# wuxiaolang/Cube_SLAM_wu

Measured on AMD Instinct MI355X. Metric: frames/sec detect_cuboid, higher is better.
Workload: dtype f64

## Files before the change

### cube_slam_wu_amd/csrc/detect_kernels.hip

```cpp
#include <hip/hip_runtime.h>
#include "cs_hip_util.h"

#include <cstdio>
#include <cstdlib>
#include <cstring>

#include "../../include/cubeslam_hip.h"
#include "detect_types.h"
#include "cs_atan2_lean.h"

namespace cs {

__device__ __forceinline__ int wave_uniform_i32(int x) { return __builtin_amdgcn_readfirstlane(x); }
__device__ __forceinline__ long long wave_uniform_i64(long long x) {
  const unsigned lo = (unsigned)__builtin_amdgcn_readfirstlane((int)(unsigned)(x & 0xffffffffll)), hi = (unsigned)__builtin_amdgcn_readfirstlane((int)(x >> 32));
  return (long long)(((unsigned long long)hi << 32) | lo);
}
__device__ __forceinline__ double wave_uniform_f64(double x) {
  int lo, hi;
  asm("v_readfirstlane_b32 %0, %1" : "=s"(lo) : "v"(__double2loint(x)));
  asm("v_readfirstlane_b32 %0, %1" : "=s"(hi) : "v"(__double2hiint(x)));
  return __hiloint2double(hi, lo);
}
template <typename T>
__device__ __forceinline__ int find_job_wave(const T* __restrict__ prefix, int n, T elem) {
  const T first = sizeof(T) == 8 ? (T)wave_uniform_i64((long long)elem) : (T)wave_uniform_i32((int)elem);
  int lo = 0, hi = n;
  while (hi - lo > 1) {
    const int mid = (lo + hi) >> 1;
    if (prefix[mid] <= first) lo = mid; else hi = mid;
  }
  while (lo + 1 < n && prefix[lo + 1] <= elem) lo++;
  return lo;
}

__device__ __forceinline__ long long xcd_virtual_block() {
  long long nb = gridDim.x, b = blockIdx.x;
  return (b & 7) * (nb >> 3) + (b >> 3);
}

__device__ __attribute__((noinline)) double vp_exact_raw(double dy, double dx) { return cs_atan2(dy, dx); }

__device__ __forceinline__ double vp_exact_unwrapped(const double* __restrict__ mx, const double* __restrict__ my, int i, int ib, double vpxk, double vpyk) {
  const double raw = vp_exact_raw(my[i] - vpyk, mx[i] - vpxk);
  if (i == ib) return raw;
  const double base = vp_exact_raw(my[ib] - vpyk, mx[ib] - vpxk);
  if ((raw - base) < -CS_PI) return raw + 2 * CS_PI;
  if ((raw - base) > CS_PI) return raw - 2 * CS_PI;
  return raw;
}
__device__ __attribute__((noinline)) float vp_rare_unwrapped_f(const double* mx, const double* my, int i, int ib, double vpxk, double vpyk) {
  return (float)vp_exact_unwrapped(mx, my, i, ib, vpxk, vpyk);
}
__device__ __attribute__((noinline)) bool vp_rare_greater(const double* mx, const double* my, int i, int i_ref, int ib, double vpxk, double vpyk) {
  return vp_exact_unwrapped(mx, my, i, ib, vpxk, vpyk) > vp_exact_unwrapped(mx, my, i_ref, ib, vpxk, vpyk);
}
__device__ __attribute__((noinline)) bool vp_rare_less(const double* mx, const double* my, int i, int i_ref, int ib, double vpxk, double vpyk) {
  return vp_exact_unwrapped(mx, my, i, ib, vpxk, vpyk) < vp_exact_unwrapped(mx, my, i_ref, ib, vpxk, vpyk);
}
struct VpExactInlier { float at; int inl; };
__device__ __attribute__((noinline)) VpExactInlier vp_rare_inlier(double dyd, double dxd, double lai, double thre) {
  const double raw = cs_atan2(dyd, dxd);
  const double nrm = normalize_to_pi(raw);
  double d = dabs(lai - nrm);
  d = dmin(d, CS_PI - d);
  return VpExactInlier{(float)raw, d < thre ? 1 : 0};
}

struct VpRun {
  bool have;
  int ib, i_hi, i_lo;
  float base_f, hi_f, lo_f;
  double hx, hy, lx, ly;
};

__device__ __forceinline__ float atan2_float(float fy, float fx, bool* usable) {
  const float PI_F = 3.14159274f, HPI_F = 1.57079637f;
  const float ay = fabsf(fy), ax = fabsf(fx);
  const float hi = fmaxf(ax, ay), lo = fminf(ax, ay);
  const float q = lo * __builtin_amdgcn_rcpf(hi), q2 = q * q;
  float at = -0.01172120f;
  at = __builtin_fmaf(at, q2, 0.05265332f);
  at = __builtin_fmaf(at, q2, -0.11643287f);
  at = __builtin_fmaf(at, q2, 0.19354346f);
  at = __builtin_fmaf(at, q2, -0.33262347f);
  at = __builtin_fmaf(at, q2, 0.99997726f);
  at = at * q;
  if (ay > ax) at = HPI_F - at;
  if (fx < 0.0f) at = PI_F - at;
  if (fy < 0.0f) at = -at;
  *usable = hi > 0.0f && hi < 3.0e38f;
  return at;
}

__device__ __forceinline__ void vp_step(const double* __restrict__ mx, const double* __restrict__ my, int i, double mxi, double myi, double lai,
                                        double vpxk, double vpyk, double thre, float thre_f, VpRun& R) {
  const float PI_F = 3.14159274f, HPI_F = 1.57079637f, M_IN = 1.0e-5f, M_ORD = 2.0e-5f;
  const double dyd = myi - vpyk, dxd = mxi - vpxk;
  bool usable;
  float at = atan2_float((float)dyd, (float)dxd, &usable);
  float nr = at;
  if (at > HPI_F) nr = at - PI_F; else if (at < -HPI_F) nr = at + PI_F;
  float df = fabsf((float)lai - nr);
  df = fminf(df, PI_F - df);
  bool inl = usable && df < thre_f - M_IN;
  if (!(inl || (usable && df > thre_f + M_IN))) { const VpExactInlier x = vp_rare_inlier(dyd, dxd, lai, thre); inl = x.inl != 0; at = x.at; }
  if (inl) {
    if (!R.have) {
      R.have = true; R.ib = i; R.i_hi = i; R.i_lo = i; R.base_f = at; R.hi_f = at; R.lo_f = at; R.hx = dxd; R.hy = dyd; R.lx = dxd; R.ly = dyd;
    } else {
      const float d = at - R.base_f;
      float sh = d < -PI_F ? at + 2.0f * PI_F : d > PI_F ? at - 2.0f * PI_F : at;
      if (fabsf(fabsf(d) - PI_F) < M_ORD) sh = vp_rare_unwrapped_f(mx, my, i, R.ib, vpxk, vpyk);
      if (sh > R.hi_f + M_ORD) { R.hi_f = sh; R.i_hi = i; R.hx = dxd; R.hy = dyd; }
      else if (sh > R.hi_f - M_ORD) {
        const double c = R.hx * dyd - R.hy * dxd, lim = 1.0e-12 * ((dabs(dxd) + dabs(dyd)) * (dabs(R.hx) + dabs(R.hy)));
        const bool greater = c > lim ? true : c < -lim ? false : vp_rare_greater(mx, my, i, R.i_hi, R.ib, vpxk, vpyk);
        if (greater) { R.hi_f = sh; R.i_hi = i; R.hx = dxd; R.hy = dyd; }
      }
      if (sh < R.lo_f - M_ORD) { R.lo_f = sh; R.i_lo = i; R.lx = dxd; R.ly = dyd; }
      else if (sh < R.lo_f + M_ORD) {
        const double c = R.lx * dyd - R.ly * dxd, lim = 1.0e-12 * ((dabs(dxd) + dabs(dyd)) * (dabs(R.lx) + dabs(R.ly)));
        const bool less = c < -lim ? true : c > lim ? false : vp_rare_less(mx, my, i, R.i_lo, R.ib, vpxk, vpyk);
        if (less) { R.lo_f = sh; R.i_lo = i; R.lx = dxd; R.ly = dyd; }
      }
    }
  }
}

struct VpChunk {
  double2 xy[64];
  double ang[64];
  float2 dir[64];
};

template <int K, bool UNIFORM>
__device__ __forceinline__ void vp_support_multi(const double* __restrict__ mx, const double* __restrict__ my, const double* __restrict__ la, int m, VpChunk* ch,
                                                 const double* vpx, const double* vpy, const double* thre, const bool* swapped, bool lane_on, double* out) {
  VpRun R[K];
  float thre_f[K], tan_f[K];
#pragma unroll
  for (int k = 0; k < K; k++) {
    R[k] = VpRun{false, 0, 0, 0, 0.f, 0.f, 0.f, 0., 0., 0., 0.}; thre_f[k] = (float)thre[k];
    tan_f[k] = thre_f[k] < 1.5f ? tanf(thre_f[k] + 1.0e-4f) : __builtin_huge_valf();
  }
  if (UNIFORM) {
    const int lane = threadIdx.x & 63;
    for (int c0 = 0; c0 < m; c0 += 64) {
      const int n = min(64, m - c0);
      __builtin_amdgcn_fence(__ATOMIC_ACQ_REL, "wavefront");
      if (lane < n) {
        const double a = la[c0 + lane];
        ch->xy[lane] = make_double2(mx[c0 + lane], my[c0 + lane]);
        ch->ang[lane] = a;
        ch->dir[lane] = make_float2(cosf((float)a), sinf((float)a));
      }
      __builtin_amdgcn_fence(__ATOMIC_ACQ_REL, "wavefront");
      __builtin_amdgcn_wave_barrier();
// ... 165 lines not shown
  int flag = 0;
  int j = find_job_wave<long long>(v.slot_prefix, v.n_jobs, active ? tid : slot_total - 1);
  const int ju = wave_uniform_i32(j);
  if (__all(j == ju)) {
    if (active) flag = candidate_one(v, sp, v.jobs[ju], tid);
  } else {
    if (active) flag = candidate_one(v, sp, v.jobs[j], tid);
  }
  unsigned long long valid = __ballot(flag != 0);
  if (valid) {
    int lane = threadIdx.x & 63;
    int j0 = __shfl(j, __ffsll((long long)valid) - 1);
    unsigned long long same = __ballot(flag != 0 && j == j0);
    if (same == valid) {
      if (lane == __ffsll((long long)valid) - 1) atomicAdd(&v.job_valid[j0], __popcll(valid));
    } else if (flag != 0) {
      atomicAdd(&v.job_valid[j], 1);
    }
  }
}

enum { COMPACT_PER = 16 };
enum { CC_TRIP = 4096 };
__global__ __launch_bounds__(256) void candidate_compact_kernel(DetectDeviceView v, SweepParams sp) {
  const int j = blockIdx.x;
  if (j >= v.n_jobs) return;
  __shared__ unsigned char s_flag[CC_TRIP];
  __shared__ int wsum[4];
  const int tid = threadIdx.x, lane = tid & 63, wid = tid >> 6;
  int jd_Y, jd_T, jd_rp_off, jd_yaw_off, jd_vp_off, jd_top_off, n_vp;
  BoxGeomD gd;
  {
    const JobDesc& jd = v.jobs[j];
    jd_Y = jd.Y; jd_T = jd.T; jd_rp_off = jd.rp_off; jd_yaw_off = jd.yaw_off; jd_vp_off = jd.vp_off; jd_top_off = jd.top_off;
    n_vp = jd.RP * jd.Y;
    const BoxGeomD g = box_geom_d(jd.g);
    gd = BoxGeomD{g.left, wave_uniform_f64(g.top), g.right, wave_uniform_f64(g.down),
                  wave_uniform_f64(g.el), wave_uniform_f64(g.et), wave_uniform_f64(g.er), wave_uniform_f64(g.eb)};
  }
  int* out_valid = v.job_valid + j;
  long long* out_cbase = v.job_cbase + j;
  asm volatile("" : "+v"(out_valid), "+v"(out_cbase));
  for (int e = tid; e < n_vp; e += 256) {
    const int rp = e / jd_Y, y = e - rp * jd_Y;
    const RpPose* pose = v.rp + jd_rp_off + rp;
    const double cy = v.yaw_cos[jd_yaw_off + y], sy = v.yaw_sin[jd_yaw_off + y];
    const double* A = pose->KinvR;
    const double d[3][3] = {{cy, sy, 0.0}, {-sy, cy, 0.0}, {0.0, 0.0, 1.0}};
    double* vout = v.vp + 6 * (long long)(jd_vp_off + e);
#pragma unroll
    for (int k = 0; k < 3; k++) {
      const double h0 = (A[0] * d[k][0] + A[1] * d[k][1]) + A[2] * d[k][2];
      const double h1 = (A[3] * d[k][0] + A[4] * d[k][1]) + A[5] * d[k][2];
      const double h2 = (A[6] * d[k][0] + A[7] * d[k][1]) + A[8] * d[k][2];
      vout[2 * k] = h0 / h2;
      vout[2 * k + 1] = h1 / h2;
    }
  }
  __syncthreads();
  const unsigned half = (unsigned)n_vp * (unsigned)jd_T;
  const unsigned Tu = (unsigned)jd_T;
  const bool fast_div = Tu > 1 && (unsigned long long)half * Tu < (1ull << 32);
  const unsigned inv_T = fast_div ? 0xffffffffu / Tu + 1u : 0u;
  const long long base = v.slot_prefix[j];
  long long run = base;
  const unsigned long long below = (1ull << lane) - 1ull;
  const bool en1 = sp.consider_config_1 != 0, en2 = sp.consider_config_2 != 0;
  const double* job_vp = v.vp + 6 * (long long)jd_vp_off;
  const int* job_top_x = v.top_x + jd_top_off;
  for (unsigned r0 = 0; r0 < half; r0 += CC_TRIP / 2) {
#pragma unroll 1
    for (int q = 0; q < 16; q++) {
      const int cfg = 1 + (q >> 3);
      const unsigned rl = (unsigned)(q & 7) * 256u + (unsigned)tid, rest = r0 + rl;
      int flag = 0;
      if (rest < half && (cfg == 1 ? en1 : en2)) {
        const unsigned ryu = fast_div ? __umulhi(rest, inv_T) : rest / Tu;
        const int t = (int)(rest - ryu * Tu);
        const double* vp = job_vp + 6 * (long long)(int)ryu;
        V2 c[8];
        flag = build_corners(gd, v2(vp[0], vp[1]), v2(vp[2], vp[3]), v2(vp[4], vp[5]), (double)job_top_x[t], cfg, sp.short_sq_bound, c);
      }
      s_flag[2 * rl + (unsigned)(cfg - 1)] = (unsigned char)flag;
    }
    __syncthreads();
    int f[COMPACT_PER];
    int wcount = 0;
#pragma unroll
    for (int q = 0; q < COMPACT_PER; q++) {
      f[q] = s_flag[wid * (64 * COMPACT_PER) + q * 64 + lane];
      wcount += __popcll(__ballot(f[q] != 0));
    }
    if (lane == 0) wsum[wid] = wcount;
    __syncthreads();
    int woff = 0, total = 0;
#pragma unroll
    for (int w = 0; w < 4; w++) { const int x = wsum[w]; if (w < wid) woff += x; total += x; }
    long long pos0 = run + woff;
    const long long sl0 = base + 2ll * r0 + wid * (64 * COMPACT_PER) + lane;
#pragma unroll
    for (int q = 0; q < COMPACT_PER; q++) {
      const unsigned long long bal = __ballot(f[q] != 0);
      if (f[q] != 0) {
        const long long pos = pos0 + __popcll(bal & below);
        v.c_slot[pos] = sl0 + q * 64;
        v.c_flag[pos] = f[q] | (j << CAND_JOB_SHIFT);
      }
      pos0 += __popcll(bal);
    }
    run += total;
    __syncthreads();
  }
  const int n_valid = (int)(run - base);
  if (tid == 0) { *out_valid = n_valid; *out_cbase = base; }
  const int nblk = (n_valid + 255) >> 8;
  if (nblk > 0) {
    __shared__ int s_at;
    if (tid == 0) s_at = atomicAdd(&v.blk_info[0], nblk);
    __syncthreads();
    const int at = s_at, b0 = (int)(base >> 8);
    for (int k = tid; k < nblk; k += 256) {
      const int left = n_valid - 256 * k;
      v.blk_info[2 + 2 * (long long)(at + k)] = b0 + k;
      v.blk_info[3 + 2 * (long long)(at + k)] = left > 256 ? 256 : left;
    }
  }
}

__device__ __forceinline__ int slot_corners(const DetectDeviceView& v, const JobDesc& jd, long long slot, double short_sq_bound, V2 c[8]) {
  const unsigned local = (unsigned)(slot - jd.slot_off);
  const unsigned rest = local >> 1, ryu = rest / (unsigned)jd.T;
  const int t = (int)(rest - ryu * (unsigned)jd.T);
  const double* vp = v.vp + 6 * (long long)(jd.vp_off + (int)ryu);
  return build_corners(jd.g, v2(vp[0], vp[1]), v2(vp[2], vp[3]), v2(vp[4], vp[5]), (double)v.top_x[jd.top_off + t], (int)(local & 1) + 1, short_sq_bound, c);
}
__device__ __forceinline__ void slot_corners16(const DetectDeviceView& v, long long slot, double short_sq_bound, double out16[16]) {
  int lo = 0, hi = v.n_jobs;
  while (hi - lo > 1) { const int mid = (lo + hi) >> 1; if (v.slot_prefix[mid] <= slot) lo = mid; else hi = mid; }
  V2 c[8];
#pragma unroll
  for (int q = 0; q < 8; q++) c[q] = v2(0.0, 0.0);
  slot_corners(v, v.jobs[lo], slot, short_sq_bound, c);
#pragma unroll
  for (int q = 0; q < 8; q++) { out16[q] = c[q].x; out16[8 + q] = c[q].y; }
}

__device__ __forceinline__ int sel(int cfg, int a, int b) { return cfg ? b : a; }

enum { SCORE_JOBS = 4, SCORE_SUB = 128, SCORE_BINS = SCORE_JOBS * SCORE_SUB };
__device__ __forceinline__ unsigned score_udiv(unsigned n, unsigned d, unsigned inv) { return inv ? __umulhi(n, inv) : n / d; }

enum { SCORE_WAVE_MIXED = 0, SCORE_WAVE_CFG1 = 1, SCORE_WAVE_CFG2 = 2 };
__device__ __forceinline__ unsigned score_sample_index(double sy, double sx, int map_w) { return (unsigned)(__mul24((int)sy, map_w) + (int)sx); }
template <int MODE>
__device__ __forceinline__ void score_edge_trip(int e0, int cfg, const double (*CXt)[260], const double (*CYt)[260], int tx, double ox, double oy,
                                                const float* __restrict__ map, int map_w, float& sum_dist) {
  const bool c2 = MODE == SCORE_WAVE_MIXED ? cfg != 0 : MODE == SCORE_WAVE_CFG2;
  const unsigned long long EA = c2 ? 0x004213210ull : 0x443213210ull, EB = c2 ? 0x005450321ull : 0x577450321ull;
  const unsigned long long EW = c2 ? 0x004332222ull : 0x222222222ull;
  const int n_edges = c2 ? 7 : 9;
  constexpr int EU = 3;
  float dv[EU][11];
#pragma unroll
  for (int u = 0; u < EU; u++) {
    const int e = e0 + u;
    if (MODE != SCORE_WAVE_MIXED && e >= n_edges) continue;
    const int a = (int)((EA >> (4 * e)) & 7), b = (int)((EB >> (4 * e)) & 7);
    const double x1 = CXt[a][tx] - ox, y1 = CYt[a][tx] - oy, x2 = CXt[b][tx] - ox, y2 = CYt[b][tx] - oy;
#pragma unroll
    for (int s = 0; s < 11; s++) {
      double sx, sy;
      if (s == 0) { sx = x2; sy = y2; }
      else if (s == 10) { sx = x1; sy = y1; }
      else if (s == 5) { sx = (x1 + x2) * 0.5; sy = (y1 + y2) * 0.5; }
      else { const double w = (double)s / 10.0; sx = w * x1 + (1 - w) * x2; sy = w * y1 + (1 - w) * y2; }
      dv[u][s] = map[score_sample_index(sy, sx, map_w)];
    }
  }
#pragma unroll
  for (int u = 0; u < EU; u++) {
    const int e = e0 + u;
    const float wt = MODE == SCORE_WAVE_CFG1 ? 1.0f : 0.5f * (float)(int)((EW >> (4 * e)) & 7);
    const bool on = e < n_edges;
    if (MODE == SCORE_WAVE_MIXED) {
#pragma unroll
      for (int s = 0; s < 11; s++) { const float nx = sum_dist + dv[u][s] * wt; sum_dist = on ? nx : sum_dist; }
    } else if (!on) {
    } else if (wt == 1.0f) {
#pragma unroll
      for (int s = 0; s < 11; s++) sum_dist += dv[u][s];
    } else {
#pragma unroll
      for (int s = 0; s < 11; s++) sum_dist += dv[u][s] * wt;
    }
  }
}
template <int MODE>
__device__ __forceinline__ float score_edge_sum(int cfg, const double (*CXt)[260], const double (*CYt)[260], int tx, double ox, double oy,
                                                const float* __restrict__ map, int map_w) {
  float sum_dist = 0;
  const int n_edges = MODE == SCORE_WAVE_MIXED ? (cfg ? 7 : 9) : MODE == SCORE_WAVE_CFG2 ? 7 : 9;
#pragma unroll 1
  for (int e0 = 0; e0 < n_edges; e0 += 3) score_edge_trip<MODE>(e0, cfg, CXt, CYt, tx, ox, oy, map, map_w, sum_dist);
  return sum_dist;
}

__device__ __forceinline__ double score_atan2(double dy, double dx, bool* accepted = nullptr) {
  double a;
  const bool ok = cs_atan2_lean(dy, dx, &a);
  if (__builtin_amdgcn_ballot_w64(!ok) != 0) {
    if (!ok) a = cs_atan2(dy, dx);
  }
  if (accepted) *accepted = ok;
  return a;
}

__global__ __launch_bounds__(256) void score_atan2_check_kernel(const double* __restrict__ y, const double* __restrict__ x, int n, double* __restrict__ out, int* __restrict__ accepted) {
  const int i = blockIdx.x * 256 + threadIdx.x;
  if (i >= n) return;
  bool ok;
  out[i] = score_atan2(y[i], x[i], &ok);
  accepted[i] = ok ? 1 : 0;
}
void launch_score_atan2_check(const double* y, const double* x, int n, double* out, int* accepted, hipStream_t st) {
  if (n <= 0) return;
  hipLaunchKernelGGL(score_atan2_check_kernel, dim3((n + 255) / 256), dim3(256), 0, st, y, x, n, out, accepted);
}

__global__ __launch_bounds__(256) void score_sample_index_check_kernel(const double* __restrict__ sy, const double* __restrict__ sx, const int* __restrict__ map_w,
                                                                       const double* __restrict__ a, const double* __restrict__ b, int n, int* __restrict__ index, double* __restrict__ probe) {
  const int i = blockIdx.x * 256 + threadIdx.x;
  if (i >= n) return;
  double pa = a[i];
  const double pb = b[i];
  const unsigned k = score_sample_index(sy[i], sx[i], map_w[i]);
  asm volatile("" : "+v"(pa) : "v"(k));
  index[i] = (int)k;
  probe[i] = pa + pb;
}
void launch_score_sample_index_check(const double* sy, const double* sx, const int* map_w, const double* a, const double* b, int n, int* index, double* probe, hipStream_t st) {
  if (n <= 0) return;
  hipLaunchKernelGGL(score_sample_index_check_kernel, dim3((n + 255) / 256), dim3(256), 0, st, sy, sx, map_w, a, b, n, index, probe);
}

template <bool CAP>
__global__ __launch_bounds__(256) void score_kernel(DetectDeviceView v, long long slot_total, double short_sq_bound) {
  __shared__ double C16[16][260];
  double (*CXt)[260] = C16, (*CYt)[260] = C16 + 8;
  const bool cap = CAP;
  long long n_valid = cap ? 256ll * v.blk_info[0] : v.job_cbase[v.n_jobs];
  const long long per_xcd = ((n_valid + 255) / 256 + 7) / 8;
  const long long kx = blockIdx.x >> 3;
  if (kx >= per_xcd) return;
  long long base = ((long long)(blockIdx.x & 7) * per_xcd + kx) * blockDim.x;
  if (base >= n_valid) return;
  if (cap) {
    const int* entry = v.blk_info + 2 + 2 * (base >> 8);
    base = 256ll * entry[0];
    n_valid = base + entry[1];
  }
  __shared__ int hist[SCORE_BINS + 1];
  __shared__ int s_src[256], s_job[256], s_flag[256];
  __shared__ long long s_slot[256];
  {
    const int t0 = threadIdx.x;
    for (int b = t0; b <= SCORE_BINS; b += 256) hist[b] = 0;
    __syncthreads();
    const long long i0 = base + t0;
    long long slot0 = 0;
    int j0 = 0;
    int flag0 = 0;
    if (i0 < n_valid) { slot0 = v.c_slot[i0]; flag0 = v.c_flag[i0]; j0 = flag0 >> CAND_JOB_SHIFT; }
    s_slot[t0] = slot0; s_job[t0] = j0; s_flag[t0] = flag0 & CAND_VP_MASK;
    __syncthreads();
    int key = SCORE_BINS;
    if (i0 < n_valid) {
      const int jq = CAP ? __builtin_amdgcn_readfirstlane(s_job[0]) : j0;
      const int T0 = v.jobs[jq].T;
      const unsigned loc = (unsigned)(slot0 - v.jobs[jq].slot_off);
      const int jrel = j0 - s_job[0];
      const unsigned hq = loc >> 1;
      const unsigned qT = CAP ? score_udiv(hq, (unsigned)T0, ((unsigned long long)v.jobs[jq].RP * v.jobs[jq].Y * T0 * T0 < (1ull << 32) && T0 > 1) ? 0xffffffffu / (unsigned)T0 + 1u : 0u) : hq / (unsigned)T0;
      const int sub = (int)(loc & 1) * T0 + (int)(hq - qT * (unsigned)T0);
      key = (jrel < SCORE_JOBS && sub < SCORE_SUB) ? jrel * SCORE_SUB + sub : SCORE_BINS - 1;
    }
    const int rank = atomicAdd(&hist[key], 1);
    __syncthreads();
    if (t0 < 64) {
      constexpr int PER = (SCORE_BINS + 1 + 63) / 64;
      int loc_sum = 0, vals[PER];
#pragma unroll
      for (int q = 0; q < PER; q++) { const int b = t0 * PER + q; vals[q] = b <= SCORE_BINS ? hist[b] : 0; loc_sum += vals[q]; }
      int incl = loc_sum;
#pragma unroll
      for (int o = 1; o < 64; o <<= 1) { const int y = __shfl_up(incl, o); if (t0 >= o) incl += y; }
      int run = incl - loc_sum;
#pragma unroll
      for (int q = 0; q < PER; q++) { const int b = t0 * PER + q; if (b <= SCORE_BINS) hist[b] = run; run += vals[q]; }
    }
    __syncthreads();
    s_src[hist[key] + rank] = t0;
    __syncthreads();
  }
  const int mine = s_src[threadIdx.x];
  const JobDesc& jd = v.jobs[CAP ? __builtin_amdgcn_readfirstlane(s_job[0]) : s_job[mine]];
  const long long i = base + mine;
  if (i >= n_valid) return;
  const long long slot = s_slot[mine];
  const unsigned local = (unsigned)(slot - jd.slot_off);
  const int cfg = (int)(local & 1);
  const unsigned inv_T = (CAP && jd.T > 1 && (unsigned long long)jd.RP * jd.Y * jd.T * jd.T < (1ull << 32)) ? 0xffffffffu / (unsigned)jd.T + 1u : 0u;
  const unsigned inv_Y = (CAP && jd.Y > 1 && (unsigned long long)jd.RP * jd.Y * jd.Y < (1ull << 32)) ? 0xffffffffu / (unsigned)jd.Y + 1u : 0u;
  const int ry = (int)score_udiv(local >> 1, (unsigned)jd.T, inv_T);
  const int rp = (int)score_udiv((unsigned)ry, (unsigned)jd.Y, inv_Y);
  const int tx = threadIdx.x;
  const double ox = (double)jd.g.el, oy = (double)jd.g.et;
  const float* __restrict__ map = v.maps + jd.map_off;
  {
    V2 cb[8];
    const unsigned rest = local >> 1;
    const double* vp = v.vp + 6 * (long long)(jd.vp_off + ry);
    rebuild_accepted_corners(jd.g, v2(vp[0], vp[1]), v2(vp[2], vp[3]), v2(vp[4], vp[5]), (double)v.top_x[jd.top_off + (int)(rest - (unsigned)ry * (unsigned)jd.T)], cfg + 1,
                             s_flag[mine], cb);
#pragma unroll
    for (int q = 0; q < 8; q++) { CXt[q][tx] = cb[q].x; CYt[q][tx] = cb[q].y; }
  }
  double bnd[6];
  {
    const double* bound = v.bound + 6 * (long long)(jd.vp_off + ry);
#pragma unroll
    for (int q = 0; q < 6; q++) bnd[q] = bound[q];
  }
  const int map_w = jd.map_w;
  const bool u1 = __all(cfg == 0), u2 = __all(cfg == 1);
  float sum_dist;
  if (u1) sum_dist = score_edge_sum<SCORE_WAVE_CFG1>(cfg, CXt, CYt, tx, ox, oy, map, map_w);
  else if (u2) sum_dist = score_edge_sum<SCORE_WAVE_CFG2>(cfg, CXt, CYt, tx, ox, oy, map, map_w);
  else sum_dist = score_edge_sum<SCORE_WAVE_MIXED>(cfg, CXt, CYt, tx, ox, oy, map, map_w);
  double total = 0;
  const double not_found_penalty = 30.0 / 180.0 * CS_PI * 2;
  const int ID1[3][4] = {{0, 1, 7, 4}, {3, 0, 4, 5}, {3, 7, 1, 5}}, ID2[3][4] = {{0, 1, 2, 3}, {3, 0, 4, 5}, {2, 4, 1, 5}};
#pragma unroll
  for (int k = 0; k < 3; k++) {
    double b0 = bnd[2 * k], b1 = bnd[2 * k + 1];
    bool v0 = !(b0 != b0), v1 = !(b1 != b1);
    if (v0 || v1) {
#pragma unroll
      for (int ee = 0; ee < 2; ee++) {
        int pa = sel(cfg, ID1[k][2 * ee], ID2[k][2 * ee]), pb = sel(cfg, ID1[k][2 * ee + 1], ID2[k][2 * ee + 1]);
        double ang = normalize_to_pi(score_atan2(CYt[pb][tx] - CYt[pa][tx], CXt[pb][tx] - CXt[pa][tx]));
        double best = 100;
        if (v0) { double t = dabs(ang - b0); t = dmin(t, CS_PI - t); if (t < best) best = t; }
        if (v1) { double t = dabs(ang - b1); t = dmin(t, CS_PI - t); if (t < best) best = t; }
        total = total + best;
      }
    } else {
      total = total + not_found_penalty;
    }
  }
  V2 c[8];
#pragma unroll
  for (int q = 0; q < 8; q++) c[q] = v2(CXt[q][tx], CYt[q][tx]);
  const RpPose* pose = v.rp + jd.rp_off + rp;
  double p3[3], s3[3];
  lift_to_3d(c, pose->R, pose->t, v.invK + 9 * jd.frame, pose->plane, p3, s3);
  int flag = s_flag[mine];
  if (s3[0] < 0 || s3[1] < 0 || s3[2] < 0) flag |= CAND_NEG_SCALE;
  v.c_flag[i] = flag;
  v.c_dist[i] = (double)sum_dist / jd.diag;
  v.c_angle[i] = total;
  v.c_skew[i] = dmax(s3[0], s3[1]) / dmin(s3[0], s3[1]);
}

__global__ __launch_bounds__(1024) void scan_jobs_kernel(const int* job_valid, long long* job_cbase, int n_jobs) {
  __shared__ long long wsum[16];
  __shared__ long long carry_s;
  if (threadIdx.x == 0) carry_s = 0;
  __syncthreads();
  int lane = threadIdx.x & 63, wid = threadIdx.x >> 6;
  for (int base = 0; base < n_jobs; base += 1024) {
    int i = base + threadIdx.x;
    long long x = (i < n_jobs) ? job_valid[i] : 0;
    long long incl = x;
#pragma unroll
    for (int o = 1; o < 64; o <<= 1) {
      long long y = __shfl_up(incl, o);
      if (lane >= o) incl += y;
    }
    if (lane == 63) wsum[wid] = incl;
    __syncthreads();
    long long woff = 0;
    for (int w = 0; w < wid; w++) woff += wsum[w];
    long long carry = carry_s;
    if (i < n_jobs) job_cbase[i] = carry + woff + incl - x;
    __syncthreads();
    if (threadIdx.x == 1023) carry_s = carry + woff + incl;
    __syncthreads();
  }
  if (threadIdx.x == 0) job_cbase[n_jobs] = carry_s;
}

__global__ __launch_bounds__(256) void compact_kernel(DetectDeviceView v) {
  int j = blockIdx.x;
  if (j >= v.n_jobs) return;
  __shared__ int wsum[4];
  const long long s0 = v.slot_prefix[j], s1 = v.slot_prefix[j + 1];
  long long run = v.job_cbase[j];
  const int lane = threadIdx.x & 63, wid = threadIdx.x >> 6;
  const unsigned long long below = (1ull << lane) - 1ull;
  for (long long base = s0; base < s1; base += 256 * COMPACT_PER) {
    const long long w0 = base + (long long)wid * (64 * COMPACT_PER) + lane;
    int f[COMPACT_PER];
    int wcount = 0;
#pragma unroll
    for (int q = 0; q < COMPACT_PER; q++) {
      const long long sl = w0 + q * 64;
      f[q] = (sl < s1) ? v.flag[sl] : 0;
      wcount += __popcll(__ballot(f[q] != 0));
    }
    if (lane == 0) wsum[wid] = wcount;
    __syncthreads();
    int woff = 0, total = 0;
#pragma unroll
    for (int w = 0; w < 4; w++) { const int x = wsum[w]; if (w < wid) woff += x; total += x; }
    long long pos0 = run + woff;
#pragma unroll
    for (int q = 0; q < COMPACT_PER; q++) {
      const unsigned long long bal = __ballot(f[q] != 0);
      if (f[q] != 0) {
        const long long pos = pos0 + __popcll(bal & below);
        v.c_slot[pos] = w0 + q * 64;
        v.c_flag[pos] = f[q] | (j << CAND_JOB_SHIFT);
      }
      pos0 += __popcll(bal);
    }
    run += total;
    __syncthreads();
  }
}

__global__ __launch_bounds__(256) void compact_count_kernel(DetectDeviceView v, int* __restrict__ cnt, int maxc) {
  const int j = blockIdx.x, c = blockIdx.y;
  __shared__ int wsum[4];
  const long long end = v.slot_prefix[j + 1], s0 = v.slot_prefix[j] + (long long)c * (256 * COMPACT_PER), s1 = (s0 + 256 * COMPACT_PER < end) ? s0 + 256 * COMPACT_PER : end;
  int n = 0;
  for (long long sl = s0 + threadIdx.x; sl < s1; sl += 256) n += v.flag[sl] != 0;
#pragma unroll
  for (int o = 32; o > 0; o >>= 1) n += __shfl_down(n, o);
  if ((threadIdx.x & 63) == 0) wsum[threadIdx.x >> 6] = n;
  __syncthreads();
  if (threadIdx.x == 0) cnt[(size_t)j * maxc + c] = wsum[0] + wsum[1] + wsum[2] + wsum[3];
}
__global__ __launch_bounds__(256) void compact_chunk_kernel(DetectDeviceView v, const int* __restrict__ cnt, int maxc) {
  const int j = blockIdx.x, c = blockIdx.y;
  __shared__ int wsum[4];
  const long long s1 = v.slot_prefix[j + 1], base = v.slot_prefix[j] + (long long)c * (256 * COMPACT_PER);
  if (base >= s1) return;
  long long run = v.job_cbase[j];
  for (int q = 0; q < c; q++) run += cnt[(size_t)j * maxc + q];
  const int lane = threadIdx.x & 63, wid = threadIdx.x >> 6;
  const unsigned long long below = (1ull << lane) - 1ull;
  const long long w0 = base + (long long)wid * (64 * COMPACT_PER) + lane;
  int f[COMPACT_PER];
  int wcount = 0;
#pragma unroll
  for (int q = 0; q < COMPACT_PER; q++) {
    const long long sl = w0 + q * 64;
    f[q] = (sl < s1) ? v.flag[sl] : 0;
    wcount += __popcll(__ballot(f[q] != 0));
  }
  if (lane == 0) wsum[wid] = wcount;
  __syncthreads();
  int woff = 0;
#pragma unroll
  for (int w = 0; w < 4; w++) if (w < wid) woff += wsum[w];
  long long pos0 = run + woff;
#pragma unroll
  for (int q = 0; q < COMPACT_PER; q++) {
    const unsigned long long bal = __ballot(f[q] != 0);
    if (f[q] != 0) {
      const long long pos = pos0 + __popcll(bal & below);
      v.c_slot[pos] = w0 + q * 64;
      v.c_flag[pos] = f[q] | (j << CAND_JOB_SHIFT);
    }
    pos0 += __popcll(bal);
  }
}

__global__ __launch_bounds__(64) void gather_corners_kernel(DetectDeviceView v, double short_sq_bound, const long long* slots, int n, double* out) {
  int w = blockIdx.x * blockDim.x + threadIdx.x;
  if (w >= n) return;
  long long s = slots[w];
  double c16[16];
#pragma unroll
  for (int q = 0; q < 16; q++) c16[q] = 0.0;
  if (s >= 0) slot_corners16(v, s, short_sq_bound, c16);
#pragma unroll
  for (int q = 0; q < 16; q++) out[16 * (size_t)w + q] = c16[q];
}


__device__ __forceinline__ unsigned long long order_key(double x) {
  unsigned long long b = (unsigned long long)__double_as_longlong(x);
  return (b >> 63) ? ~b : (b | 0x8000000000000000ull);
}

template <int NT>
__device__ void block_radix_select2(const double* __restrict__ a, const double* __restrict__ b, int n, int r, unsigned* hist , unsigned long long* bcast ,
                                    unsigned long long* key_a, unsigned long long* key_b) {
  unsigned long long prefix[2] = {0, 0}, mask = 0;
  int rr2[2] = {r, r};
  for (int pass = 0; pass < 8; pass++) {
    const int shift = 56 - 8 * pass;
    for (int q = threadIdx.x; q < 512; q += NT) hist[q] = 0;
    __syncthreads();
    for (int i = threadIdx.x; i < n; i += NT) {
      const unsigned long long ka = order_key(a[i]), kb = order_key(b[i]);
      if ((ka & mask) == prefix[0]) atomicAdd(&hist[(unsigned)(ka >> shift) & 255u], 1u);
      if ((kb & mask) == prefix[1]) atomicAdd(&hist[256 + ((unsigned)(kb >> shift) & 255u)], 1u);
// ... 1228 lines not shown
```

Before: 575,600.

## Shrink score kernel LDS footprint and dedupe corner map samples for higher occupancy

Stores corner y-values for corners 0 and 4 as wave-uniform scalars (top/down) rather than in shared memory, cutting corner rows from 16 to 14. In CAP mode it also shrinks the histogram, slot, job and flag arrays. Uniform-config paths are fully unrolled per edge group, with each corner's map sample loaded once and reused as the shared edge endpoint. Launch bounds request five waves in CAP mode, and the bound loads move after the edge sum. The changes rely on the geometric invariant that those corners share top/down y, and add register pressure and complexity.

```diff
diff --git a/cube_slam_wu_amd/csrc/detect_kernels.hip b/cube_slam_wu_amd/csrc/detect_kernels.hip
--- a/cube_slam_wu_amd/csrc/detect_kernels.hip
+++ b/cube_slam_wu_amd/csrc/detect_kernels.hip
@@ -4,6 +4,7 @@
 #include <cstdio>
 #include <cstdlib>
 #include <cstring>
+#include <type_traits>
 
 #include "../../include/cubeslam_hip.h"
 #include "detect_types.h"
@@ -475,41 +476,106 @@
 
 enum { SCORE_WAVE_MIXED = 0, SCORE_WAVE_CFG1 = 1, SCORE_WAVE_CFG2 = 2 };
 __device__ __forceinline__ unsigned score_sample_index(double sy, double sx, int map_w) { return (unsigned)(__mul24((int)sy, map_w) + (int)sx); }
-template <int MODE>
-__device__ __forceinline__ void score_edge_trip(int e0, int cfg, const double (*CXt)[260], const double (*CYt)[260], int tx, double ox, double oy,
-                                                const float* __restrict__ map, int map_w, float& sum_dist) {
-  const bool c2 = MODE == SCORE_WAVE_MIXED ? cfg != 0 : MODE == SCORE_WAVE_CFG2;
-  const unsigned long long EA = c2 ? 0x004213210ull : 0x443213210ull, EB = c2 ? 0x005450321ull : 0x577450321ull;
-  const unsigned long long EW = c2 ? 0x004332222ull : 0x222222222ull;
+
+enum { SCORE_LD = 260, SCORE_XROWS = 8, SCORE_YROWS = 6, SCORE_ROWS = SCORE_XROWS + SCORE_YROWS };
+enum { SCORE_WAVES = 5 };
+enum { SCORE_TOP = -1, SCORE_DOWN = -2 };
+__host__ __device__ constexpr int score_xrow(int c) { return c; }
+__host__ __device__ constexpr int score_yrow(int c) { return c == 0 ? (int)SCORE_TOP : c == 4 ? (int)SCORE_DOWN : SCORE_XROWS + c - 1 - (c > 4 ? 1 : 0); }
+__device__ __forceinline__ double score_uniform_f64(double x) {
+  int lo, hi;
+  asm("s_nop 0\n\tv_readfirstlane_b32 %0, %2\n\tv_readfirstlane_b32 %1, %3\n\ts_nop 1" : "=s"(lo), "=s"(hi) : "v"(__double2loint(x)), "v"(__double2hiint(x)));
+  return __hiloint2double(hi, lo);
+}
+struct ScoreCorners {
+  double (*R)[SCORE_LD];
+  int tx;
+  double top, down;
+  __device__ __forceinline__ double row(int r) const { return r == SCORE_TOP ? +top : r == SCORE_DOWN ? +down : +R[r][tx]; }
+  __device__ __forceinline__ double x(int c) const { return row(score_xrow(c)); }
+  __device__ __forceinline__ double y(int c) const { return row(score_yrow(c)); }
+  __device__ __forceinline__ double pick(int r1, int r2, int cfg) const { return r1 == r2 ? row(r1) : (r1 >= 0 && r2 >= 0) ? +R[cfg ? r2 : r1][tx] : cfg ? row(r2) : row(r1); }
+  __device__ __forceinline__ double x_of(int c1, int c2, int cfg) const { return pick(score_xrow(c1), score_xrow(c2), cfg); }
+  __device__ __forceinline__ double y_of(int c1, int c2, int cfg) const { return pick(score_yrow(c1), score_yrow(c2), cfg); }
+  __device__ __forceinline__ double x_dyn(int c) const { return R[c][tx]; }
+  __device__ __forceinline__ double y_dyn(int c) const {
+    const double s = R[SCORE_XROWS + (c == 0 || c == 4 ? 0 : c - 1 - (c > 4 ? 1 : 0))][tx], t = top, d = down;
+    return c == 0 ? +t : c == 4 ? +d : +s;
+  }
+  template <int Q>
+  __device__ __forceinline__ void store_corner(const V2& p) {
+    if (score_yrow(Q) >= 0) R[score_yrow(Q)][tx] = p.y;
+    R[score_xrow(Q)][tx] = p.x;
+  }
+  __device__ __forceinline__ void store(const V2 (&cb)[8]) {
+    store_corner<0>(cb[0]); store_corner<1>(cb[1]); store_corner<2>(cb[2]); store_corner<3>(cb[3]);
+    store_corner<4>(cb[4]); store_corner<5>(cb[5]); store_corner<6>(cb[6]); store_corner<7>(cb[7]);
+  }
+};
+
+__host__ __device__ constexpr unsigned long long score_edge_a(bool c2) { return c2 ? 0x004213210ull : 0x443213210ull; }
+__host__ __device__ constexpr unsigned long long score_edge_b(bool c2) { return c2 ? 0x005450321ull : 0x577450321ull; }
+__host__ __device__ constexpr unsigned long long score_edge_w(bool c2) { return c2 ? 0x004332222ull : 0x222222222ull; }
+__device__ __forceinline__ unsigned score_edge_sample(int s, double x1, double y1, double x2, double y2, int map_w) {
+  double sx, sy;
+  if (s == 0) { sx = x2; sy = y2; }
+  else if (s == 10) { sx = x1; sy = y1; }
+  else if (s == 5) { sx = (x1 + x2) * 0.5; sy = (y1 + y2) * 0.5; }
+  else { const double w = (double)s / 10.0; sx = w * x1 + (1 - w) * x2; sy = w * y1 + (1 - w) * y2; }
+  return score_sample_index(sy, sx, map_w);
+}
+__host__ __device__ constexpr bool score_corner_ends_edge(int c, bool c2) {
+  for (int e = 0; e < (c2 ? 7 : 9); e++) if ((int)((score_edge_a(c2) >> (4 * e)) & 7) == c || (int)((score_edge_b(c2) >> (4 * e)) & 7) == c) return true;
+  return false;
+}
+constexpr int SCORE_EU = 3;
+
+__device__ __forceinline__ void score_edge_trip_mixed(int e0, int cfg, const ScoreCorners& K, double ox, double oy, const float* __restrict__ map, int map_w, float& sum_dist) {
+  const bool c2 = cfg != 0;
+  const unsigned long long EA = c2 ? score_edge_a(true) : score_edge_a(false), EB = c2 ? score_edge_b(true) : score_edge_b(false);
+  const unsigned long long EW = c2 ? score_edge_w(true) : score_edge_w(false);
   const int n_edges = c2 ? 7 : 9;
-  constexpr int EU = 3;
-  float dv[EU][11];
-#pragma unroll
-  for (int u = 0; u < EU; u++) {
+  float dv[SCORE_EU][11];
+#pragma unroll
+  for (int u = 0; u < SCORE_EU; u++) {
     const int e = e0 + u;
-    if (MODE != SCORE_WAVE_MIXED && e >= n_edges) continue;
     const int a = (int)((EA >> (4 * e)) & 7), b = (int)((EB >> (4 * e)) & 7);
-    const double x1 = CXt[a][tx] - ox, y1 = CYt[a][tx] - oy, x2 = CXt[b][tx] - ox, y2 = CYt[b][tx] - oy;
-#pragma unroll
-    for (int s = 0; s < 11; s++) {
-      double sx, sy;
-      if (s == 0) { sx = x2; sy = y2; }
-      else if (s == 10) { sx = x1; sy = y1; }
-      else if (s == 5) { sx = (x1 + x2) * 0.5; sy = (y1 + y2) * 0.5; }
-      else { const double w = (double)s / 10.0; sx = w * x1 + (1 - w) * x2; sy = w * y1 + (1 - w) * y2; }
-      dv[u][s] = map[score_sample_index(sy, sx, map_w)];
-    }
-  }
-#pragma unroll
-  for (int u = 0; u < EU; u++) {
+    const double x1 = K.x_dyn(a) - ox, y1 = K.y_dyn(a) - oy, x2 = K.x_dyn(b) - ox, y2 = K.y_dyn(b) - oy;
+#pragma unroll
+    for (int s = 0; s < 11; s++) dv[u][s] = map[score_edge_sample(s, x1, y1, x2, y2, map_w)];
+  }
+#pragma unroll
+  for (int u = 0; u < SCORE_EU; u++) {
     const int e = e0 + u;
-    const float wt = MODE == SCORE_WAVE_CFG1 ? 1.0f : 0.5f * (float)(int)((EW >> (4 * e)) & 7);
+    const float wt = 0.5f * (float)(int)((EW >> (4 * e)) & 7);
     const bool on = e < n_edges;
-    if (MODE == SCORE_WAVE_MIXED) {
-#pragma unroll
-      for (int s = 0; s < 11; s++) { const float nx = sum_dist + dv[u][s] * wt; sum_dist = on ? nx : sum_dist; }
-    } else if (!on) {
-    } else if (wt == 1.0f) {
+#pragma unroll
+    for (int s = 0; s < 11; s++) { const float nx = sum_dist + dv[u][s] * wt; sum_dist = on ? nx : sum_dist; }
+  }
+}
+template <bool C2, int E0>
+__device__ __forceinline__ void score_edge_trip(const ScoreCorners& K0, const float (&cv)[8], double ox, double oy, const float* __restrict__ map, int map_w, float& sum_dist) {
+  constexpr int n_edges = C2 ? 7 : 9;
+  ScoreCorners K = K0;
+  asm volatile("" : "+v"(K.tx));
+  float dv[SCORE_EU][11];
+#pragma unroll
+  for (int u = 0; u < SCORE_EU; u++) {
+    const int e = E0 + u;
+    if (e >= n_edges) continue;
+    const int a = (int)((score_edge_a(C2) >> (4 * e)) & 7), b = (int)((score_edge_b(C2) >> (4 * e)) & 7);
+    const double x1 = K.x(a) - ox, y1 = K.y(a) - oy, x2 = K.x(b) - ox, y2 = K.y(b) - oy;
+    dv[u][0] = cv[b]; dv[u][10] = cv[a];
+#pragma unroll
+    for (int s = 1; s < 10; s++) dv[u][s] = map[score_edge_sample(s, x1, y1, x2, y2, map_w)];
+    __builtin_amdgcn_sched_barrier(0);
+  }
+#pragma unroll
+  for (int u = 0; u < SCORE_EU; u++) {
+    const int e = E0 + u;
+    if (e >= n_edges) continue;
+    const float wt = 0.5f * (float)(int)((score_edge_w(C2) >> (4 * e)) & 7);
+    if (wt == 1.0f) {
 #pragma unroll
       for (int s = 0; s < 11; s++) sum_dist += dv[u][s];
     } else {
@@ -519,12 +585,27 @@
   }
 }
 template <int MODE>
-__device__ __forceinline__ float score_edge_sum(int cfg, const double (*CXt)[260], const double (*CYt)[260], int tx, double ox, double oy,
-                                                const float* __restrict__ map, int map_w) {
+__device__ __forceinline__ float score_edge_sum(int cfg, const ScoreCorners& K, double ox, double oy, const float* __restrict__ map, int map_w) {
   float sum_dist = 0;
-  const int n_edges = MODE == SCORE_WAVE_MIXED ? (cfg ? 7 : 9) : MODE == SCORE_WAVE_CFG2 ? 7 : 9;
+  if (MODE == SCORE_WAVE_MIXED) {
+    const int n_edges = cfg ? 7 : 9;
 #pragma unroll 1
-  for (int e0 = 0; e0 < n_edges; e0 += 3) score_edge_trip<MODE>(e0, cfg, CXt, CYt, tx, ox, oy, map, map_w, sum_dist);
+    for (int e0 = 0; e0 < n_edges; e0 += SCORE_EU) score_edge_trip_mixed(e0, cfg, K, ox, oy, map, map_w, sum_dist);
+  } else {
+    constexpr bool C2 = MODE == SCORE_WAVE_CFG2;
+    float cv[8];
+#pragma unroll
+    for (int c = 0; c < 8; c++) {
+      const bool used = score_corner_ends_edge(c, C2);
+      cv[c] = used ? map[score_sample_index(K.y(c) - oy, K.x(c) - ox, map_w)] : 0.0f;
+    }
+    score_edge_trip<C2, 0>(K, cv, ox, oy, map, map_w, sum_dist);
+    __builtin_amdgcn_sched_barrier(0);
+    score_edge_trip<C2, SCORE_EU>(K, cv, ox, oy, map, map_w, sum_dist);
+    __builtin_amdgcn_sched_barrier(0);
+    score_edge_trip<C2, 2 * SCORE_EU>(K, cv, ox, oy, map, map_w, sum_dist);
+    __builtin_amdgcn_sched_barrier(0);
+  }
   return sum_dist;
 }
 
@@ -567,9 +648,8 @@
 }
 
 template <bool CAP>
-__global__ __launch_bounds__(256) void score_kernel(DetectDeviceView v, long long slot_total, double short_sq_bound) {
-  __shared__ double C16[16][260];
-  double (*CXt)[260] = C16, (*CYt)[260] = C16 + 8;
+__global__ __launch_bounds__(256, CAP ? SCORE_WAVES : 4) void score_kernel(DetectDeviceView v, long long slot_total, double short_sq_bound) {
+  __shared__ double s_rows[SCORE_ROWS][SCORE_LD];
   const bool cap = CAP;
   long long n_valid = cap ? 256ll * v.blk_info[0] : v.job_cbase[v.n_jobs];
   const long long per_xcd = ((n_valid + 255) / 256 + 7) / 8;
@@ -582,84 +662,91 @@
     base = 256ll * entry[0];
     n_valid = base + entry[1];
   }
-  __shared__ int hist[SCORE_BINS + 1];
-  __shared__ int s_src[256], s_job[256], s_flag[256];
-  __shared__ long long s_slot[256];
+  constexpr int NBINS = CAP ? (int)SCORE_SUB : (int)SCORE_BINS;
+  using SlotT = typename std::conditional<CAP, unsigned, long long>::type;
+  __shared__ int hist[NBINS + 1];
+  __shared__ unsigned char s_src[256], s_flag[256];
+  __shared__ int s_job[CAP ? 1 : 256];
+  __shared__ SlotT s_slot[256];
   {
     const int t0 = threadIdx.x;
-    for (int b = t0; b <= SCORE_BINS; b += 256) hist[b] = 0;
+    for (int b = t0; b <= NBINS; b += 256) hist[b] = 0;
     __syncthreads();
     const long long i0 = base + t0;
     long long slot0 = 0;
     int j0 = 0;
     int flag0 = 0;
     if (i0 < n_valid) { slot0 = v.c_slot[i0]; flag0 = v.c_flag[i0]; j0 = flag0 >> CAND_JOB_SHIFT; }
-    s_slot[t0] = slot0; s_job[t0] = j0; s_flag[t0] = flag0 & CAND_VP_MASK;
-    __syncthreads();
-    int key = SCORE_BINS;
+    const int jq = CAP ? __builtin_amdgcn_readfirstlane(j0) : j0;
+    const unsigned loc = (unsigned)(slot0 - v.jobs[jq].slot_off);
+    if (CAP) { s_slot[t0] = (SlotT)loc; if (t0 == 0) s_job[0] = j0; }
+    else { s_slot[t0] = (SlotT)slot0; s_job[t0] = j0; }
+    s_flag[t0] = (unsigned char)(flag0 & CAND_VP_MASK);
+    __syncthreads();
+    int key = NBINS;
     if (i0 < n_valid) {
-      const int jq = CAP ? __builtin_amdgcn_readfirstlane(s_job[0]) : j0;
       const int T0 = v.jobs[jq].T;
-      const unsigned loc = (unsigned)(slot0 - v.jobs[jq].slot_off);
-      const int jrel = j0 - s_job[0];
+      const int jrel = CAP ? 0 : j0 - s_job[0];
       const unsigned hq = loc >> 1;
       const unsigned qT = CAP ? score_udiv(hq, (unsigned)T0, ((unsigned long long)v.jobs[jq].RP * v.jobs[jq].Y * T0 * T0 < (1ull << 32) && T0 > 1) ? 0xffffffffu / (unsigned)T0 + 1u : 0u) : hq / (unsigned)T0;
       const int sub = (int)(loc & 1) * T0 + (int)(hq - qT * (unsigned)T0);
-      key = (jrel < SCORE_JOBS && sub < SCORE_SUB) ? jrel * SCORE_SUB + sub : SCORE_BINS - 1;
+      key = (jrel < (CAP ? 1 : (int)SCORE_JOBS) && sub < SCORE_SUB) ? jrel * SCORE_SUB + sub : NBINS - 1;
     }
     const int rank = atomicAdd(&hist[key], 1);
     __syncthreads();
     if (t0 < 64) {
-      constexpr int PER = (SCORE_BINS + 1 + 63) / 64;
+      constexpr int PER = (NBINS + 1 + 63) / 64;
       int loc_sum = 0, vals[PER];
 #pragma unroll
-      for (int q = 0; q < PER; q++) { const int b = t0 * PER + q; vals[q] = b <= SCORE_BINS ? hist[b] : 0; loc_sum += vals[q]; }
+      for (int q = 0; q < PER; q++) { const int b = t0 * PER + q; vals[q] = b <= NBINS ? hist[b] : 0; loc_sum += vals[q]; }
       int incl = loc_sum;
 #pragma unroll
       for (int o = 1; o < 64; o <<= 1) { const int y = __shfl_up(incl, o); if (t0 >= o) incl += y; }
       int run = incl - loc_sum;
 #pragma unroll
-      for (int q = 0; q < PER; q++) { const int b = t0 * PER + q; if (b <= SCORE_BINS) hist[b] = run; run += vals[q]; }
-    }
-    __syncthreads();
-    s_src[hist[key] + rank] = t0;
+      for (int q = 0; q < PER; q++) { const int b = t0 * PER + q; if (b <= NBINS) hist[b] = run; run += vals[q]; }
+    }
+    __syncthreads();
+    s_src[hist[key] + rank] = (unsigned char)t0;
     __syncthreads();
   }
   const int mine = s_src[threadIdx.x];
   const JobDesc& jd = v.jobs[CAP ? __builtin_amdgcn_readfirstlane(s_job[0]) : s_job[mine]];
   const long long i = base + mine;
   if (i >= n_valid) return;
-  const long long slot = s_slot[mine];
-  const unsigned local = (unsigned)(slot - jd.slot_off);
+  const unsigned local = CAP ? (unsigned)s_slot[mine] : (unsigned)((long long)s_slot[mine] - jd.slot_off);
   const int cfg = (int)(local & 1);
   const unsigned inv_T = (CAP && jd.T > 1 && (unsigned long long)jd.RP * jd.Y * jd.T * jd.T < (1ull << 32)) ? 0xffffffffu / (unsigned)jd.T + 1u : 0u;
   const unsigned inv_Y = (CAP && jd.Y > 1 && (unsigned long long)jd.RP * jd.Y * jd.Y < (1ull << 32)) ? 0xffffffffu / (unsigned)jd.Y + 1u : 0u;
   const int ry = (int)score_udiv(local >> 1, (unsigned)jd.T, inv_T);
   const int rp = (int)score_udiv((unsigned)ry, (unsigned)jd.Y, inv_Y);
   const int tx = threadIdx.x;
-  const double ox = (double)jd.g.el, oy = (double)jd.g.et;
+  const double ox = CAP ? score_uniform_f64((double)jd.g.el) : (double)jd.g.el, oy = CAP ? score_uniform_f64((double)jd.g.et) : (double)jd.g.et;
   const float* __restrict__ map = v.maps + jd.map_off;
+  const int kept = s_flag[mine];
+  ScoreCorners K;
+  K.R = s_rows; K.tx = tx;
+  K.top = CAP ? score_uniform_f64((double)jd.g.top) : (double)jd.g.top; K.down = CAP ? score_uniform_f64((double)jd.g.down) : (double)jd.g.down;
   {
     V2 cb[8];
     const unsigned rest = local >> 1;
     const double* vp = v.vp + 6 * (long long)(jd.vp_off + ry);
     rebuild_accepted_corners(jd.g, v2(vp[0], vp[1]), v2(vp[2], vp[3]), v2(vp[4], vp[5]), (double)v.top_x[jd.top_off + (int)(rest - (unsigned)ry * (unsigned)jd.T)], cfg + 1,
-                             s_flag[mine], cb);
-#pragma unroll
-    for (int q = 0; q < 8; q++) { CXt[q][tx] = cb[q].x; CYt[q][tx] = cb[q].y; }
-  }
+                             kept, cb);
+    K.store(cb);
+  }
+  const int map_w = jd.map_w;
+  const bool u1 = __all(cfg == 0), u2 = __all(cfg == 1);
+  float sum_dist;
+  if (u1) sum_dist = score_edge_sum<SCORE_WAVE_CFG1>(cfg, K, ox, oy, map, map_w);
+  else if (u2) sum_dist = score_edge_sum<SCORE_WAVE_CFG2>(cfg, K, ox, oy, map, map_w);
+  else sum_dist = score_edge_sum<SCORE_WAVE_MIXED>(cfg, K, ox, oy, map, map_w);
   double bnd[6];
   {
     const double* bound = v.bound + 6 * (long long)(jd.vp_off + ry);
 #pragma unroll
     for (int q = 0; q < 6; q++) bnd[q] = bound[q];
   }
-  const int map_w = jd.map_w;
-  const bool u1 = __all(cfg == 0), u2 = __all(cfg == 1);
-  float sum_dist;
-  if (u1) sum_dist = score_edge_sum<SCORE_WAVE_CFG1>(cfg, CXt, CYt, tx, ox, oy, map, map_w);
-  else if (u2) sum_dist = score_edge_sum<SCORE_WAVE_CFG2>(cfg, CXt, CYt, tx, ox, oy, map, map_w);
-  else sum_dist = score_edge_sum<SCORE_WAVE_MIXED>(cfg, CXt, CYt, tx, ox, oy, map, map_w);
   double total = 0;
   const double not_found_penalty = 30.0 / 180.0 * CS_PI * 2;
   const int ID1[3][4] = {{0, 1, 7, 4}, {3, 0, 4, 5}, {3, 7, 1, 5}}, ID2[3][4] = {{0, 1, 2, 3}, {3, 0, 4, 5}, {2, 4, 1, 5}};
@@ -670,8 +757,8 @@
     if (v0 || v1) {
 #pragma unroll
       for (int ee = 0; ee < 2; ee++) {
-        int pa = sel(cfg, ID1[k][2 * ee], ID2[k][2 * ee]), pb = sel(cfg, ID1[k][2 * ee + 1], ID2[k][2 * ee + 1]);
-        double ang = normalize_to_pi(score_atan2(CYt[pb][tx] - CYt[pa][tx], CXt[pb][tx] - CXt[pa][tx]));
+        const int pa1 = ID1[k][2 * ee], pa2 = ID2[k][2 * ee], pb1 = ID1[k][2 * ee + 1], pb2 = ID2[k][2 * ee + 1];
+        double ang = normalize_to_pi(score_atan2(K.y_of(pb1, pb2, cfg) - K.y_of(pa1, pa2, cfg), K.x_of(pb1, pb2, cfg) - K.x_of(pa1, pa2, cfg)));
         double best = 100;
         if (v0) { double t = dabs(ang - b0); t = dmin(t, CS_PI - t); if (t < best) best = t; }
         if (v1) { double t = dabs(ang - b1); t = dmin(t, CS_PI - t); if (t < best) best = t; }
@@ -683,11 +770,11 @@
   }
   V2 c[8];
 #pragma unroll
-  for (int q = 0; q < 8; q++) c[q] = v2(CXt[q][tx], CYt[q][tx]);
+  for (int q = 0; q < 8; q++) c[q] = (q == 1 || q >= 4) ? v2(K.x(q), K.y(q)) : v2(0.0, 0.0);
   const RpPose* pose = v.rp + jd.rp_off + rp;
   double p3[3], s3[3];
   lift_to_3d(c, pose->R, pose->t, v.invK + 9 * jd.frame, pose->plane, p3, s3);
-  int flag = s_flag[mine];
+  int flag = kept;
   if (s3[0] < 0 || s3[1] < 0 || s3[2] < 0) flag |= CAND_NEG_SCALE;
   v.c_flag[i] = flag;
   v.c_dist[i] = (double)sum_dist / jd.diag;
```

After: 576,900, median of 2. No clear change (+0.2%).
